# peterrum/dealii-multigrid

Measured on AMD Instinct MI355X. Metric: DoF/s per V-cycle, 3D octant p=4, higher is better.
Workload: dtype f64; 1 GPU; 3D octant (GeometryType quadrant) HMG-global p=4 FP64, NRefGlobal=8, SmootherDegree=3, coarse solver direct, f=1, zero Dirichlet (BASELINE.json configs[2]); n_dofs=137199985, n_cells=2127189, n_levels=9, parallelism=1 GPU, chebyshev_start_vector=deal.II's (i mod 11) - mean on the local numbering, fused_transfer_bricks=33509

## Files before the change

### dealii_multigrid_amd/csrc/kernels_apply.hpp

```cpp
#pragma once
#include "kernels_common.hpp"

namespace mgamd
{
#ifdef MGAMD_KERNEL_DEBUG
#define MGAMD_STAMP(k)                         \
  if (args.stamps && tid == 0)                 \
    args.stamps[(size_t)block * 8 + (k)] = wall_clock64();
#define MGAMD_ABLATED(bit) (args.ablate & (bit))
#else
#define MGAMD_STAMP(k)
#define MGAMD_ABLATED(bit) false
#endif

  template <typename T, int P, int B, int MODE, bool CONSTR = false, bool WAVE = false>
  __device__ __forceinline__ void
  lattice_apply_body(const ApplyArgs<T, P> &args, const uint32_t block, const uint32_t nblocks, unsigned char *smem_raw)
  {
    static_assert(!WAVE || (B == 1 && !CONSTR), "wave-scoped slots: single cells");
    using G  = Geo<P, B, WAVE ? 64 : 256>;
    using IM = InteriorMap<P, B, WAVE ? 64 : 256>;
    T *bufA = reinterpret_cast<T *>(smem_raw);
    T *bufB = bufA + G::SPW * G::N3;

// ... 196 lines not shown
      {
        any_hanging = __syncthreads_or((int)(fm_early != 0)) != 0;
        if (any_hanging)
          brick_constraint_passes<T, P, B, BLOCK>(bufA, args.m, tid, nslots, args.g.fmask + slot0, false, G::ROUNDS == 1 ? &fm_line : nullptr);
      }
    MGAMD_STAMP(5)

    if (!MGAMD_ABLATED(1))
      {
        if constexpr (G::ROUNDS == 1)
          lattice_sweeps<T, P, B, BLOCK, NoHook, false, false, WAVE>(bufA, bufB, args.m, tid, nslots, &h_mine, NoHook(), true);
        else
          lattice_sweeps<T, P, B, BLOCK, NoHook, false, false, WAVE>(bufA, bufB, args.m, tid, nslots, args.g.h + slot0);
      }
    MGAMD_STAMP(6)

    if (B == 1 && any_hanging)
      hanging_passes<T, P, WAVE>(bufA, args.m, sl, u, v, act, mask, true);
    if constexpr (brick_may_be_constrained(B, CONSTR))
      if (any_hanging)
        brick_constraint_passes<T, P, B, BLOCK>(bufA, args.m, tid, nslots, args.g.fmask + slot0, true, G::ROUNDS == 1 ? &fm_line : nullptr);
    MGAMD_STAMP(2)

    if (G::N_INT > 0 && !MGAMD_ABLATED(4))
      {
#pragma unroll
        for (int it = 0; it < ITER; ++it)
          if (const Ent e = ent(it); e.l >= 0)
            {
              const T ax = bufA[e.l];
              T       r;
              if (MODE == MODE_VMULT)
                r = ax;
              else if (MODE == MODE_RESIDUAL)
                r = bv[it] - ax;
              else
                {
                  const T dv  = CLOSED_DINV ? interior_dinv(it) : dvm[CLOSED_DINV ? 0 : it];
                  const T xov = MODE == MODE_CHEB_SECOND ? args.epi.c0 * dv * bv[it] : xo[it];
                  r           = xg[it] + args.epi.f1 * (xg[it] - xov) + args.epi.f2 * dv * (bv[it] - ax);
                }
              if (MODE == MODE_CHEB)
                store_result(args.epi, e.g, r);
              else
                NT_STORE(r, &args.epi.out[e.g]);
            }
      }
    MGAMD_STAMP(3)
    if (!MGAMD_ABLATED(2))
      {
#pragma unroll
        for (int it = 0; it < ITERS; ++it)
          if (spos[it] >= 0 && sgi[it] < args.scatter_limit)
            atomic_add(&args.tail_acc[sgi[it] - args.n_interior], bufA[spos[it]]);
      }
#ifdef MGAMD_KERNEL_DEBUG
    if (args.stamps)
      {
        __builtin_amdgcn_s_waitcnt(0);
        slot_sync<WAVE>();
        MGAMD_STAMP(4)
      }
#endif
  }

  template <typename T, int P, int B, int MODE_, bool CONSTR = false>
  __device__ __forceinline__ void
  lattice_apply_persistent_body(const ApplyArgs<T, P> &args, const uint32_t w, const uint32_t stride, unsigned char *smem_raw)
  {
    using G  = Geo<P, B>;
    using IM = InteriorMap<P, B>;
    static_assert(G::SPW == 1 && G::N_INT > 0, "persistent workgroups: one slot per workgroup");
    constexpr int  MODE   = base_mode(MODE_);
    constexpr bool FUSE_R = MODE_ == MODE_RESIDUAL_RESTRICT, FUSE_P = MODE_ == MODE_CHEB_PROLONGATE, FUSE = FUSE_R || FUSE_P;
    static_assert(!FUSE || (!CONSTR && B >= 2 && G::ABLOCK == 256), "fused transfers: plain bricks, 256 threads");
    constexpr int BC = B >= 2 ? B / 2 : 1, NC = P * BC + 1, NC3 = NC * NC * NC;
    T *bufA = reinterpret_cast<T *>(smem_raw);
    T *bufB = bufA + G::N3;
    T *dtab = bufB + G::N3;
    T *Etab = dtab + 2 * P * P * P + 1;
    constexpr bool FACE_PASSES = CONSTR && P >= 2 && B > 2 && face_table_words<P, B>() > 0 && G::N * (G::N - 2) <= G::ABLOCK;

    constexpr int BLOCK = G::ABLOCK;
    constexpr int ITER  = (G::N_INT + BLOCK - 1) / BLOCK;
    constexpr int ITERS = (G::N_SHELL + BLOCK - 1) / BLOCK;
    constexpr int ITC   = FUSE ? (NC3 + BLOCK - 1) / BLOCK : 1;
    constexpr int P3    = P * P * P;
    static_assert(!FUSE || 2 * ITERS <= 15, "two flag bits per shell entry in a 16-bit word");

    const int      tid = threadIdx.x;
    const uint32_t n   = args.g.n_slots;
    if (w >= n)
      return;

    if constexpr (FACE_PASSES)
      for (int t = tid; t < (2 * P + 1) * (P + 1); t += BLOCK)
        {
          const int a = t / (P + 1), b = t % (P + 1);
          Etab[t]     = a <= P ? args.m.I0[a * (P + 1) + b] : args.m.I1[(a - P) * (P + 1) + b];
        }
    if (is_cheb(MODE))
      {
        for (int t = tid; t < P3; t += BLOCK)
          {
            const int tt[3] = {t % P, (t / P) % P, t / (P * P)};
            T         m[3], k[3];
#pragma unroll
// ... 304 lines not shown
                  }
                __syncthreads();
                for (int l = tid; l < NC * NC; l += BLOCK)
                  {
                    const int b0 = (l / NC) * G::N + l % NC;
#pragma unroll
                    for (int i = 0; i < G::N; ++i)
                      rin[i] = bufA[b0 + i * G::N * G::N];
                    line_embed_sym_T<T, P, BC>(args.fused.Eh, rin, rout);
#pragma unroll
                    for (int i = 0; i < NC; ++i)
                      bufB[l + i * NC * NC] = rout[i];
                  }
                __syncthreads();
#pragma unroll
                for (int it = 0; it < ITC; ++it)
                  if (tid + it * BLOCK < NC3 && cgi[it] != DEV_INVALID)
                    atomic_add(&args.fused.coarse[cgi[it]], bufB[tid + it * BLOCK]);
              }
          }
        else
          {
            InteriorWalk wk = walk0;
#pragma unroll
            for (int it = 0; it < ITER; ++it, wk.next())
              if (has_entry(it))
                {
                  const uint32_t g  = base + (uint32_t)(tid + it * BLOCK);
                  const T        ax = bufA[wk.pos()];
                  T              r;
                  if (MODE == MODE_VMULT)
                    r = ax;
                  else if (MODE == MODE_RESIDUAL)
                    r = bv[it] - ax;
                  else
                    {
                      const T dv  = interior_dinv(wk.type());
                      const T xov = MODE == MODE_CHEB_SECOND ? args.epi.c0 * dv * bv[it] : xo[it];
                      const T xv  = x_from_b ? args.epi.c0 * dv * bv[it] : xg[it];
                      if (FUSE_P)
                        r = xv + args.epi.f2 * dv * (bv[it] - ax);
                      else
                        r = xv + args.epi.f1 * (xv - xov) + args.epi.f2 * dv * (bv[it] - ax);
                    }
                  if (MODE == MODE_CHEB && !FUSE_P)
                    store_result(args.epi, g, r);
                  else
                    NT_STORE(r, &args.epi.out[g]);
                }
            MGAMD_STAMP(3)
#pragma unroll
            for (int it = 0; it < ITERS; ++it)
              if (spos[it] >= 0 && sgi[it] < args.scatter_limit)
                atomic_add(&args.tail_acc[sgi[it] - args.n_interior], bufA[spos[it]]);
          }
        MGAMD_STAMP(4)
        if (!has_next)
          break;
        v    = vn;
        slot  = slotn;
        base  = basen;
        hcur  = hn;
        fmcur = fmn;
        flcur = fln;
#pragma unroll
        for (int it = 0; it < ITC; ++it)
          {
            cgi[it]  = cgn[it];
            cval[it] = cvaln[it];
          }
#pragma unroll
        for (int it = 0; it < ITERS; ++it)
          {
            sgi[it]  = sgn[it];
            sval[it] = svaln[it];
            sb[it]   = sbn[it];
          }
#pragma unroll
        for (int it = 0; it < ITER; ++it)
          xg[it] = xgn[it];
        __syncthreads();
      }
  }
#undef MGAMD_STAMP
#undef MGAMD_ABLATED

  template <typename T, int P, int B, int MODE, bool CONSTR = false>
  __global__ void
  __launch_bounds__((Geo<P, B>::ABLOCK), (Geo<P, B>::ROUNDS > 1 ? 2 : (B == 1 ? 6 : (B == 2 ? 4 : 1)))) lattice_apply_kernel(const ApplyArgs<T, P> args)
  {
    extern __shared__ __align__(16) unsigned char smem_raw[];
    lattice_apply_body<T, P, B, MODE, CONSTR>(args, blockIdx.x, gridDim.x, smem_raw);
  }

  constexpr int CELL_WAVES = 4;
  template <typename T, int P>
  constexpr size_t
  cell_wave_lds()
  {
    using G = Geo<P, 1, 64>;
    return (((2 * (size_t)G::SPW * G::N3 + 2 * P * P * P + G::SPW) * sizeof(T) + 15) / 16) * 16;
  }
  template <typename T, int P, int MODE>
  __device__ __forceinline__ void
  cell_waves_body(const ApplyArgs<T, P> &args, const uint32_t block, const uint32_t nblocks, unsigned char *smem_raw)
  {
    const uint32_t wave = threadIdx.x >> 6;
// ... 70 lines not shown
        a.stamps          = nullptr;
        lattice_apply_persistent_body<T, P, B, base_mode(MODE), true>(a, blockIdx.x - args.n_wg_plain, gridDim.x - args.n_wg_plain, smem_raw);
      }
  }

  template <typename T, int P>
  struct SmallSlotsArgs
  {
    ApplyArgs<T, P> a;
    SlotGroupDev    g_cells;
    uint32_t        n_wg_bricks;
  };
  template <typename T, int P, int MODE>
  __global__ void
  __launch_bounds__(256, 4) lattice_apply_small_kernel(const SmallSlotsArgs<T, P> args)
  {
    extern __shared__ __align__(16) unsigned char smem_raw[];
    if (blockIdx.x < args.n_wg_bricks)
      lattice_apply_body<T, P, 2, MODE>(args.a, blockIdx.x, args.n_wg_bricks, smem_raw);
    else
      {
        ApplyArgs<T, P> a = args.a;
        a.g               = args.g_cells;
        a.stamps          = nullptr;
        cell_waves_body<T, P, MODE>(a, blockIdx.x - args.n_wg_bricks, gridDim.x - args.n_wg_bricks, smem_raw);
      }
  }

  struct CellClusterDev
  {
    const uint32_t *uniq_ptr;
    const uint32_t *uniq_idx;
    const uint16_t *loc;
    const uint16_t *mask;
    const double   *h;
    uint32_t        n_slots;
    uint32_t        max_uniq;
  };
  constexpr int CLUSTER_CELLS = 256;
  constexpr int CLUSTER_ITERS = 8;

  template <typename T>
  struct ClusterArgs
  {
    CellClusterDev c;
    Mats<1, T>     m;
    const T       *src;
    T             *tail_acc;
    uint32_t       n_interior;
    const T *b, *dinv;
    T        c0;
    int      from_b;
    uint32_t cluster_offset;
  };

  template <typename T, bool TRANSPOSE>
  __device__ __forceinline__ void
  hanging_in_registers_p1(T (&x)[8], const uint32_t mask, const Mats<1, T> &m)
  {
    const int  cx = mask & 1, cy = (mask >> 1) & 1, cz = (mask >> 2) & 1;
    const bool fx = (mask >> 3) & 1, fy = (mask >> 4) & 1, fz = (mask >> 5) & 1;
    const bool ex = (mask >> 6) & 1, ey = (mask >> 7) & 1, ez = (mask >> 8) & 1;
#pragma unroll
    for (int dd = 0; dd < 3; ++dd)
      {
        const int d = TRANSPOSE ? 2 - dd : dd;
#pragma unroll
        for (int v = 0; v < 2; ++v)
#pragma unroll
          for (int u = 0; u < 2; ++u)
            {
              bool on;
              int  c;
              if (d == 0)
                {
                  const bool ou = u == cy, ov = v == cz;
                  on            = (fy && ou) || (fz && ov) || (ex && ou && ov);
                  c             = cx;
                }
              else if (d == 1)
                {
                  const bool ou = u == cx, ov = v == cz;
                  on            = (fx && ou) || (fz && ov) || (ey && ou && ov);
                  c             = cy;
                }
              else
                {
                  const bool ou = u == cx, ov = v == cy;
                  on            = (fx && ou) || (fy && ov) || (ez && ou && ov);
                  c             = cz;
                }
              const int i0 = d == 0 ? (v * 2 + u) * 2 : (d == 1 ? v * 4 + u : v * 2 + u);
              const int i1 = i0 + (d == 0 ? 1 : (d == 1 ? 2 : 4));
              if (on)
                {
                  const T *w       = c ? m.I1 : m.I0;
                  const T       a0 = x[i0], a1 = x[i1];
                  if (TRANSPOSE)
                    {
                      x[i0] = T(w[0]) * a0 + T(w[2]) * a1;
                      x[i1] = T(w[1]) * a0 + T(w[3]) * a1;
                    }
                  else
                    {
                      x[i0] = T(w[0]) * a0 + T(w[1]) * a1;
                      x[i1] = T(w[2]) * a0 + T(w[3]) * a1;
// ... 65 lines not shown
    T             x[8];
#pragma unroll
    for (int i = 0; i < 8; ++i)
      {
        l[i] = (lw4[i / 2] >> (16 * (i % 2))) & 0xFFFFu;
        x[i] = (act && l[i] != 0xFFFFu) ? U[l[i]] : T(0);
      }
    if (mask >> 3)
      hanging_in_registers_p1<T, false>(x, mask, a.m);
    const T M0 = T(a.m.M[0]), M1 = T(a.m.M[1]), M2 = T(a.m.M[2]), M3 = T(a.m.M[3]);
    const T K0 = T(a.m.K[0]), K1 = T(a.m.K[1]), K2 = T(a.m.K[2]), K3 = T(a.m.K[3]);
    T       A[8], Bv[8];
#pragma unroll
    for (int q = 0; q < 4; ++q)
      {
        const T r0 = x[q], r1 = x[q + 4];
        A[q]       = M0 * r0 + M1 * r1;
        A[q + 4]   = M2 * r0 + M3 * r1;
        Bv[q]      = K0 * r0 + K1 * r1;
        Bv[q + 4]  = K2 * r0 + K3 * r1;
      }
#pragma unroll
    for (int q = 0; q < 4; ++q)
      {
        const int i0 = (q & 1) + 4 * (q >> 1);
        const T   a0 = A[i0], a1 = A[i0 + 2], b0 = Bv[i0], b1 = Bv[i0 + 2];
        A[i0]        = M0 * a0 + M1 * a1;
        A[i0 + 2]    = M2 * a0 + M3 * a1;
        Bv[i0]       = K0 * a0 + K1 * a1 + M0 * b0 + M1 * b1;
        Bv[i0 + 2]   = K2 * a0 + K3 * a1 + M2 * b0 + M3 * b1;
      }
#pragma unroll
    for (int q = 0; q < 4; ++q)
      {
        const T a0 = A[2 * q], a1 = A[2 * q + 1], b0 = Bv[2 * q], b1 = Bv[2 * q + 1];
        x[2 * q]     = h * (K0 * a0 + K1 * a1 + M0 * b0 + M1 * b1);
        x[2 * q + 1] = h * (K2 * a0 + K3 * a1 + M2 * b0 + M3 * b1);
      }
    if (mask >> 3)
      hanging_in_registers_p1<T, true>(x, mask, a.m);
    if (act)
      {
#pragma unroll
        for (int i = 0; i < 8; ++i)
          if (l[i] != 0xFFFFu)
            atomic_add(&Acc[l[i]], x[i]);
      }
    __syncthreads();
#pragma unroll
    for (int k = 0; k < CLUSTER_ITERS; ++k)
      {
        const int j = tid + k * CLUSTER_CELLS;
        if (j < nu)
          atomic_add(&a.tail_acc[gi[k] - a.n_interior], Acc[j]);
      }
  }

  template <typename T>
  __global__ void
  __launch_bounds__(CLUSTER_CELLS) cell_cluster_apply_kernel(const ClusterArgs<T> a)
  {
    extern __shared__ __align__(16) unsigned char smem_raw[];
    cell_cluster_body<T>(a, blockIdx.x, gridDim.x, smem_raw);
  }

  template <typename T>
  struct P1SmallArgs
  {
    ApplyArgs<T, 1> a;
    ClusterArgs<T>  c;
    uint32_t        n_wg_bricks;
  };
  template <typename T, int MODE>
  __global__ void
  __launch_bounds__(256) lattice_cluster_kernel(const P1SmallArgs<T> args)
  {
    extern __shared__ __align__(16) unsigned char smem_raw[];
    if (blockIdx.x < args.n_wg_bricks)
      lattice_apply_body<T, 1, 8, MODE>(args.a, blockIdx.x, args.n_wg_bricks, smem_raw);
    else
      cell_cluster_body<T>(args.c, blockIdx.x - args.n_wg_bricks, gridDim.x - args.n_wg_bricks, smem_raw);
  }

  template <typename T, int P, int B, bool CONSTR = false>
  __global__ void
  __launch_bounds__((Geo<P, B>::BLOCK)) lattice_diag_kernel(const ApplyArgs<T, P> args)
  {
    using G = Geo<P, B>;
    extern __shared__ __align__(16) unsigned char smem_raw[];
    T *bufA = reinterpret_cast<T *>(smem_raw);
    T *bufB = bufA + G::SPW * G::N3;
    T *bufD = bufB + G::SPW * G::N3;

    const int tid    = threadIdx.x;
    const int slot0  = blockIdx.x * G::SPW;
    const int nslots = min((int)G::SPW, (int)args.g.n_slots - slot0);
    const int sl     = tid / G::LINES;
    const int ln     = tid % G::LINES;
    const int u = ln % G::N, v = ln / G::N;
    const bool act = tid < G::SPW * G::LINES && sl < nslots;

    uint32_t mask = 0;
    T        h    = T(0);
    if (act)
      {
        h = T(args.g.h[slot0 + sl]);
        if (B == 1)
// ... 39 lines not shown
        if (any_hanging)
          for (int j = 0; j < G::N3; ++j)
            {
              for (int idx = tid; idx < G::SPW * G::N3; idx += G::BLOCK)
                bufA[idx] = (idx % G::N3) == j ? T(1) : T(0);
              __syncthreads();
              hanging_passes<T, P>(bufA, args.m, sl, u, v, act, mask, false);
              lattice_sweeps<T, P, B, G::BLOCK>(bufA, bufB, args.m, tid, nslots, args.g.h + slot0);
              hanging_passes<T, P>(bufA, args.m, sl, u, v, act, mask, true);
              if (act && ln == 0 && (mask >> 3))
                bufD[sl * G::N3 + j] = bufA[sl * G::N3 + j];
              __syncthreads();
            }
      }
    if constexpr (brick_may_be_constrained(B, CONSTR))
      {
        uint32_t fm = 0;
        if (args.g.fmask != nullptr && tid < nslots)
          fm = args.g.fmask[slot0 + tid];
        const bool any_family = __syncthreads_or((int)(fm != 0)) != 0;
        if (any_family)
          for (int s = 0; s < G::N_SHELL; ++s)
            {
              const int j = args.g.shell_pos[s];
              for (int idx = tid; idx < G::SPW * G::N3; idx += G::BLOCK)
                bufA[idx] = (idx % G::N3) == j ? T(1) : T(0);
              __syncthreads();
              brick_constraint_passes<T, P, B, G::BLOCK>(bufA, args.m, tid, nslots, args.g.fmask + slot0, false);
              lattice_sweeps<T, P, B, G::BLOCK>(bufA, bufB, args.m, tid, nslots, args.g.h + slot0);
              brick_constraint_passes<T, P, B, G::BLOCK>(bufA, args.m, tid, nslots, args.g.fmask + slot0, true);
              if (act && ln == 0 && args.g.fmask[slot0 + sl])
                bufD[sl * G::N3 + j] = bufA[sl * G::N3 + j];
              __syncthreads();
            }
      }
    if (G::N_INT > 0)
      for (int idx = tid; idx < nslots * G::N_INT; idx += G::BLOCK)
        {
          const int sl2 = idx / (G::N_INT > 0 ? G::N_INT : 1), i = idx % (G::N_INT > 0 ? G::N_INT : 1);
          const int x = i % (G::NI > 0 ? G::NI : 1), y = (i / (G::NI > 0 ? G::NI : 1)) % (G::NI > 0 ? G::NI : 1),
                    z = i / (G::NI > 0 ? G::NI * G::NI : 1);
          const T d = bufD[sl2 * G::N3 + ((z + 1) * G::N + (y + 1)) * G::N + x + 1];
          apply_epilogue<T, MODE_INVDIAG>(args.epi, args.g.interior_base[slot0 + sl2] + i, d);
        }
    for (int idx = tid; idx < nslots * G::N_SHELL; idx += G::BLOCK)
      {
        const int      sl2 = idx / G::N_SHELL, s = idx % G::N_SHELL;
        const uint32_t gi  = args.g.shell_idx[(size_t)(slot0 + sl2) * G::N_SHELL + s];
        if (gi < args.scatter_limit)
          atomic_add(&args.tail_acc[gi - args.n_interior], bufD[sl2 * G::N3 + args.g.shell_pos[s]]);
      }
  }

  template <typename T, int MODE_>
  __global__ void
  __launch_bounds__(256) tail_kernel(T *__restrict__ tail_acc, uint32_t n_interior, uint32_t n_tail, uint32_t n_rest, Epilogue<T> epi)
  {
    constexpr int  MODE   = base_mode(MODE_);
    constexpr bool FUSE_P = MODE_ == MODE_CHEB_PROLONGATE;
    constexpr int  U      = 4;
    const uint32_t total  = n_tail + n_rest;
    const uint32_t stride = gridDim.x * blockDim.x;
    __shared__ T   dtable[256];
    const bool     coded = is_cheb(MODE) && epi.dinv_code != nullptr;
    if (coded)
      {
        dtable[threadIdx.x] = epi.dinv_table[threadIdx.x];
        __syncthreads();
      }
    for (uint32_t i0 = blockIdx.x * blockDim.x + threadIdx.x; i0 < total; i0 += U * stride)
      {
        T ax[U], xv[U], xo[U], bv[U], dv[U];
#pragma unroll
        for (int u = 0; u < U; ++u)
          {
            const uint32_t i  = i0 + u * stride;
            const uint32_t gi = n_interior + i;
            ax[u] = xv[u] = xo[u] = bv[u] = dv[u] = T(0);
            if (i < total)
              {
                if (MODE != MODE_INVDIAG && MODE != MODE_CHEB_FIRST && (is_cheb(MODE) || i >= n_tail))
                  {
                    if (FUSE_P && i < n_tail && NT_LOAD(&epi.xs_flag[i]))
                      {
                        xv[u] = NT_LOAD(&epi.xs[gi]);
                        epi.x_inout[gi] = xv[u];
                      }
                    else
                      xv[u] = NT_LOAD(&epi.x[gi]);
                  }
                ax[u] = i < n_tail ? tail_acc[i] : xv[u];
                if (MODE == MODE_RESIDUAL || is_cheb(MODE))
                  bv[u] = NT_LOAD(&epi.b[gi]);
                if (is_cheb(MODE))
                  {
                    if (MODE == MODE_CHEB && epi.xold)
                      xo[u] = NT_LOAD(&epi.xold[gi]);
                    if (coded)
                      {
                        const uint32_t c = NT_LOAD(&epi.dinv_code[i]);
                        dv[u]            = c != 255u ? dtable[c] : epi.dinv[gi];
                      }
                    else
                      dv[u] = epi.dinv[gi];
                  }
              }
          }
#pragma unroll
        for (int u = 0; u < U; ++u)
          {
            const uint32_t i  = i0 + u * stride;
            const uint32_t gi = n_interior + i;
            if (i < total)
              {
                if (i < n_tail)
                  NT_STORE(T(0), &tail_acc[i]);
                if (MODE == MODE_CHEB_FIRST || MODE == MODE_CHEB_SECOND)
                  {
                    const T x1 = epi.c0 * dv[u] * bv[u];
                    if (MODE == MODE_CHEB_FIRST)
                      {
                        xv[u] = x1;
                        if (i >= n_tail)
                          ax[u] = x1;
                      }
                    else
                      xo[u] = x1;
                  }
                if (MODE == MODE_VMULT)
                  NT_STORE(ax[u], &epi.out[gi]);
                else if (MODE == MODE_RESIDUAL)
                  NT_STORE(bv[u] - ax[u], &epi.out[gi]);
                else if (is_cheb(MODE))
                  {
                    const T r = xv[u] + epi.f1 * (xv[u] - xo[u]) + epi.f2 * dv[u] * (bv[u] - ax[u]);
                    if (MODE_ == MODE_CHEB)
                      store_result(epi, gi, r);
                    else
                      NT_STORE(r, &epi.out[gi]);
                  }
                else
                  epi.out[gi] = (i < n_tail && fabs((double)ax[u]) > 1.0e-10) ? T(1) / ax[u] : T(1);
              }
          }
      }
  }

}
```

### dealii_multigrid_amd/csrc/kernels_common.hpp

```cpp
#pragma once
#include <hip/hip_runtime.h>
#include <stdint.h>

namespace mgamd
{
  constexpr uint32_t DEV_INVALID = 0xFFFFFFFFu;

#ifndef MGAMD_NO_NT_STREAMS
#define NT_LOAD(p) __builtin_nontemporal_load(p)
#define NT_STORE(v, p) __builtin_nontemporal_store(v, p)
#else
#define NT_LOAD(p) (*(p))
#define NT_STORE(v, p) (*(p) = (v))
#endif

  __device__ __forceinline__ uint32_t
  xcd_contiguous(uint32_t b, uint32_t n)
  {
    const uint32_t k = b & 7u, q = n >> 3, r = n & 7u;
    return k * q + (k < r ? k : r) + (b >> 3);
  }

  template <int P, typename S = double>
  struct Mats
// ... 66 lines not shown
    T        f1, f2;
    T        c0;
    const uint8_t *dinv_code  = nullptr;
    const T       *dinv_table = nullptr;
    const uint8_t *xs_flag = nullptr;
    const T       *xs      = nullptr;
    T             *x_inout = nullptr;
    double *out_wide = nullptr;
  };
  template <typename T>
  __device__ __forceinline__ void
  store_result(const Epilogue<T> &e, const uint32_t g, const T r)
  {
    if (sizeof(T) == 4 && e.out_wide != nullptr)
      __builtin_nontemporal_store((double)r, &e.out_wide[g]);
    else
      __builtin_nontemporal_store(r, &e.out[g]);
  }
  constexpr bool
  is_cheb(int mode)
  {
    return mode == MODE_CHEB || mode == MODE_CHEB_FIRST || mode == MODE_CHEB_SECOND;
  }

  template <typename T, int MODE>
  __device__ __forceinline__ void
  apply_epilogue(const Epilogue<T> &e, uint32_t gi, T Ax)
  {
    if (MODE == MODE_VMULT)
      e.out[gi] = Ax;
    else if (MODE == MODE_RESIDUAL)
      e.out[gi] = e.b[gi] - Ax;
    else if (MODE == MODE_CHEB)
      {
        const T xv = e.x[gi];
        const T xo = e.xold ? e.xold[gi] : T(0);
        e.out[gi]  = xv + e.f1 * (xv - xo) + e.f2 * e.dinv[gi] * (e.b[gi] - Ax);
      }
    else
      e.out[gi] = (fabs((double)Ax) > 1.0e-10) ? T(1) / Ax : T(1);
  }

  __device__ __forceinline__ void
  atomic_add(double *p, double v)
  {
    unsafeAtomicAdd(p, v);
  }
  __device__ __forceinline__ void
  atomic_add(float *p, float v)
  {
    unsafeAtomicAdd(p, v);
  }

  template <typename T, int P, int B>
  __device__ __forceinline__ void
  line_mult(const T *__restrict__ Mc, const T (&in)[P * B + 1], T (&out)[P * B + 1])
  {
#pragma unroll
    for (int i = 0; i < P * B + 1; ++i)
      out[i] = T(0);
#pragma unroll
    for (int c = 0; c < B; ++c)
#pragma unroll
      for (int a = 0; a <= P; ++a)
#pragma unroll
        for (int b = 0; b <= P; ++b)
          out[c * P + a] += T(Mc[a * (P + 1) + b]) * in[c * P + b];
  }

  template <typename T, int P>
  struct EvenOdd
  {
    static constexpr int NH = (P + 2) / 2, NO = (P + 1) / 2;
    T                    e[NH], o[NO];
    __device__ __forceinline__ void
    split(const T *x)
    {
#pragma unroll
      for (int j = 0; j < NO; ++j)
        {
          e[j] = x[j] + x[P - j];
          o[j] = x[j] - x[P - j];
        }
      if (NH > NO)
        e[NH - 1] = x[NH - 1];
    }
    template <bool ACC>
    __device__ __forceinline__ void
    apply(const T *__restrict__ Ae, const T *__restrict__ Ao, const EvenOdd &x)
    {
#pragma unroll
      for (int i = 0; i < NH; ++i)
        {
          T acc = ACC ? e[i] : T(0);
#pragma unroll
          for (int j = 0; j < NH; ++j)
            acc += T(Ae[i * NH + j]) * x.e[j];
          e[i] = acc;
        }
#pragma unroll
      for (int i = 0; i < NO; ++i)
        {
          T acc = ACC ? o[i] : T(0);
#pragma unroll
          for (int j = 0; j < NO; ++j)
            acc += T(Ao[i * NO + j]) * x.o[j];
// ... 826 lines not shown
```

### dealii_multigrid_amd/csrc/level_operator.hpp

```cpp
#pragma once
#include "runtime.hpp"
#include "kernels.hpp"

#include <cmath>
#include <cstring>
#include <map>
#include <mutex>
#include <type_traits>
#include <unordered_map>

namespace mgamd
{
  inline int
  grid_for(size_t n)
  {
    size_t g = (n + 255) / 256;
    if (g > 2048)
      g = 2048;
    if (g < 1)
      g = 1;
    return (int)g;
  }

  template <typename T>
// ... 365 lines not shown
                           halo->sh_owner_src.p, nsh);
      HIP_CHECK(hipGetLastError());
    }
    void
    exchange_add_tail(mgamd_vec &v) override
    {
      if (v.n != n_dofs())
        throw std::invalid_argument("exchange_add_tail: vector size mismatch");
      exchange_add_raw(v.as<T>() + tables->n_interior);
    }
    double
    dot_raw_global(const T *x, const T *y)
    {
      if (!comm)
        return dot_raw(ctx, x, y, (size_t)n_dofs());
      const double local = dot_raw(ctx, x, y, (size_t)tables->n_interior + tables->n_tail_owned);
      return comm->allreduce_sum_host(local, ctx->stream);
    }
    double
    dot(const mgamd_vec &x, const mgamd_vec &y) override
    {
      if (x.n != n_dofs() || y.n != n_dofs())
        throw std::invalid_argument("dot: vector size mismatch");
      return dot_raw_global(x.as<T>(), y.as<T>());
    }

    template <int P>
    Mats<P, T>
    mats() const
    {
      Mats<P, T> m;
      const int n = P + 1;
      for (int i = 0; i < n * n; ++i)
        {
          m.M[i]  = tables->fe.M[i];
          m.K[i]  = tables->fe.K[i];
          m.I0[i] = tables->fe.I[0][i];
          m.I1[i] = tables->fe.I[1][i];
        }
      constexpr int NH = Mats<P>::NH, NO = Mats<P>::NO;
      auto          eo = [&](const double *A, T *Ae, T *Ao) {
        for (int i = 0; i < NH; ++i)
          for (int j = 0; j < NH; ++j)
            Ae[i * NH + j] = (j < NO) ? 0.5 * (A[i * n + j] + A[i * n + P - j]) : A[i * n + j];
        for (int i = 0; i < NO; ++i)
          for (int j = 0; j < NO; ++j)
            Ao[i * NO + j] = 0.5 * (A[i * n + j] - A[i * n + P - j]);
      };
      eo(tables->fe.M.data(), m.Me, m.Mo);
      eo(tables->fe.K.data(), m.Ke, m.Ko);
      return m;
    }

    ClusterArgs<T>
    cluster_args(const GroupDev<T> &g, const T *src, const Epilogue<T> &epi, bool first)
    {
      ClusterArgs<T> a;
      a.c          = g.cluster_view();
      a.m          = mats<1>();
      a.src        = src;
      a.tail_acc   = tail_acc.p;
      a.n_interior = tables->n_interior;
      a.b          = epi.b;
      a.dinv       = epi.dinv;
      a.c0         = epi.c0;
      a.from_b     = first ? 1 : 0;
      a.cluster_offset = 0;
      return a;
    }

    void
    launch_clusters(hipStream_t st, const GroupDev<T> &g, const T *src, const Epilogue<T> &epi, bool first, uint32_t cluster_begin = 0,
                    uint32_t cluster_end = 0xFFFFFFFFu)
    {
      ClusterArgs<T> a;
      a.c          = g.cluster_view();
      a.m          = mats<1>();
      a.src        = src;
      a.tail_acc   = tail_acc.p;
      a.n_interior = tables->n_interior;
      a.b          = epi.b;
      a.dinv       = epi.dinv;
      a.c0         = epi.c0;
      a.from_b     = first ? 1 : 0;
      a.cluster_offset = 0;
      const uint32_t n_cl = (uint32_t)((g.n_slots + CLUSTER_CELLS - 1) / CLUSTER_CELLS);
      cluster_end         = std::min(cluster_end, n_cl);
      if (cluster_begin >= cluster_end)
        return;
      a.cluster_offset    = cluster_begin;
      const uint32_t grid = cluster_end - cluster_begin;
      hipLaunchKernelGGL(cell_cluster_apply_kernel<T>, grid, CLUSTER_CELLS, 2 * (size_t)std::max<uint32_t>(g.max_uniq, 1) * sizeof(T), st, a);
      HIP_CHECK(hipGetLastError());
    }

    template <int P, int B, int MODE>
    void
    launch_pair(hipStream_t st, const ApplyArgs<T, P> &a, GroupDev<T> *g_constrained)
    {
      using G = Geo<P, B>;
      BrickPairArgs<T, P> pa;
      pa.a             = a;
      pa.g_constrained = g_constrained->view();
      pa.n_wg_plain    = (uint32_t)((a.g.n_slots + G::SPW - 1) / G::SPW);
      const uint32_t n_wg_c = (uint32_t)((g_constrained->n_slots + G::SPW - 1) / G::SPW);
      const size_t   lds    = (2 * (size_t)G::SPW * G::N3 + 2 * P * P * P + G::SPW + face_table_words<P, B>()) * sizeof(T);
      if constexpr (G::SPW == 1 && G::N_INT > 0 && G::ROUNDS > 1)
        if (use_persistent<T, P>())
          {
            const int resident = resident_workgroups(ctx);
            uint32_t  np = pa.n_wg_plain, nc = n_wg_c;
            if ((int)(np + nc) > resident)
              {
                np = 0;
                nc = (uint32_t)resident;
              }
            pa.n_wg_plain = np;
            auto kern     = lattice_apply_persistent_pair_kernel<T, P, B, MODE>;
            ensure_dynamic_lds(ctx, reinterpret_cast<const void *>(kern), lds);
            hipLaunchKernelGGL(kern, np + nc, G::ABLOCK, lds, st, pa);
            HIP_CHECK(hipGetLastError());
            return;
          }
      if constexpr (MODE != base_mode(MODE))
        throw std::runtime_error("fused transfers need the persistent brick kernel");
      else
        {
          auto kern = lattice_apply_pair_kernel<T, P, B, MODE>;
          ensure_dynamic_lds(ctx, reinterpret_cast<const void *>(kern), lds);
          hipLaunchKernelGGL(kern, pa.n_wg_plain + n_wg_c, G::ABLOCK, lds, st, pa);
          HIP_CHECK(hipGetLastError());
        }
    }

    template <int P, int MODE>
    void
    launch_fused(hipStream_t st, ApplyArgs<T, P> &a, size_t begin, GroupDev<T> *partner_constrained, const FusedTransferHost<T> &f)
    {
// ... 13 lines not shown
              if (std::fabs(f.E[(2 * P - ar) * (P + 1) + (P - b)] - f.E[ar * (P + 1) + b]) > 1e-14)
                throw std::runtime_error("fused transfer: the 1D embedding is not centro-symmetric");
          a.fused.coarse  = f.coarse;
          a.fused.x_inout = f.x_inout;
          a.fused.scratch = f.scratch;
          if (partner_constrained)
            {
              if constexpr (P == 1)
                return launch_pair<P, B, MODE>(st, a, partner_constrained);
              throw std::runtime_error("brick pair launch: size not instantiated");
            }
          const size_t lds      = (2 * (size_t)G::N3 + 2 * P * P * P + 1 + face_table_words<P, B>()) * sizeof(T);
          const int    resident = resident_workgroups(ctx, persistent_wgs_per_cu<T, P>());
          auto         kern     = lattice_apply_persistent_kernel<T, P, B, MODE>;
          ensure_dynamic_lds(ctx, reinterpret_cast<const void *>(kern), lds);
          hipLaunchKernelGGL(kern, std::min((int)a.g.n_slots, resident), G::ABLOCK, lds, st, a);
          HIP_CHECK(hipGetLastError());
        }
      else
        throw std::runtime_error("fused transfers: degree without 17-point lattice kernel");
    }

    template <int P, int MODE_>
    void
    launch_group(hipStream_t st, ApplyArgs<T, P> &a, GroupDev<T> *g, GroupDev<T> *partner_cells, GroupDev<T> *partner_clusters,
                 const T *src, const Epilogue<T> &epi, bool diag, size_t begin, size_t end, GroupDev<T> *partner_constrained = nullptr,
                 const FusedTransferHost<T> *fused = nullptr)
    {
      constexpr int MODE = base_mode(MODE_);
      a.g      = (begin == 0 && end == g->n_slots) ? g->view() : g->view(begin, end);
      if constexpr (MODE_ != MODE)
        if (fused && fused->group >= 0 && g == groups[fused->group].get())
          return launch_fused<P, MODE_>(st, a, begin, partner_constrained, *fused);
      if (partner_constrained)
        {
          if constexpr (P == 1)
            {
              if (g->B == 16)
                return launch_pair<P, 16, MODE>(st, a, partner_constrained);
              if (g->B == 8)
                return launch_pair<P, 8, MODE>(st, a, partner_constrained);
            }
          throw std::runtime_error("brick pair launch: size not instantiated");
        }
      a.stamps = (stamps.p && g->B == prof_B && !g->constrained && MODE == stamp_mode && !diag && begin == 0) ? stamps.p : nullptr;
      if (partner_clusters)
        {
          if constexpr (P == 1)
            {
              using G8 = Geo<1, 8>;
              GroupDev<T>   *gc = partner_clusters;
              P1SmallArgs<T> sa;
              sa.a           = a;
              sa.c           = cluster_args(*gc, src, epi, MODE == MODE_CHEB_FIRST);
              sa.n_wg_bricks = (uint32_t)((g->n_slots + G8::SPW - 1) / G8::SPW);
              const uint32_t n_wg_cl = (uint32_t)((gc->n_slots + CLUSTER_CELLS - 1) / CLUSTER_CELLS);
              const size_t   lds     = std::max((2 * (size_t)G8::SPW * G8::N3 + 2 + G8::SPW) * sizeof(T),
                                          2 * (size_t)std::max<uint32_t>(gc->max_uniq, 1) * sizeof(T));
              hipLaunchKernelGGL((lattice_cluster_kernel<T, MODE>), sa.n_wg_bricks + n_wg_cl, 256, lds, st, sa);
              HIP_CHECK(hipGetLastError());
            }
        }
      else if (P == 1 && !diag && g->has_clusters())
        launch_clusters(st, *g, src, epi, MODE == MODE_CHEB_FIRST);
      else if (partner_cells)
        {
          if constexpr (P >= 2)
            {
              using G2 = Geo<P, 2>;
              using G1 = Geo<P, 1>;
              GroupDev<T>         *g1 = partner_cells;
              SmallSlotsArgs<T, P> sa;
              sa.a           = a;
              sa.g_cells     = g1->view();
              sa.n_wg_bricks = (uint32_t)((g->n_slots + G2::SPW - 1) / G2::SPW);
              using GW = Geo<P, 1, 64>;
              const uint32_t n_w        = (uint32_t)((g1->n_slots + GW::SPW - 1) / GW::SPW);
              const uint32_t n_wg_cells = (n_w + CELL_WAVES - 1) / CELL_WAVES;
              const size_t   lds        = std::max((2 * (size_t)G2::SPW * G2::N3 + 2 * P * P * P + G2::SPW) * sizeof(T), CELL_WAVES * cell_wave_lds<T, P>());
              (void)sizeof(G1);
              hipLaunchKernelGGL((lattice_apply_small_kernel<T, P, MODE>), sa.n_wg_bricks + n_wg_cells, 256, lds, st, sa);
              HIP_CHECK(hipGetLastError());
            }
        }
      else
        dispatch_B<T, P, MODE>(ctx, st, g->B, g->constrained, a, diag);
    }

    template <int MODE>
    void
    launch_tail(hipStream_t st, uint32_t begin, uint32_t end, bool with_rest, const Epilogue<T> &epi_in, bool diag)
    {
      const uint32_t n_rest = with_rest ? tables->n_dofs - tables->n_interior - end : 0;
      const uint32_t n_t    = end - begin + n_rest;
      if (!n_t)
        return;
      Epilogue<T> epi = epi_in;
      if (epi.dinv_code)
        epi.dinv_code += begin;
      if (diag)
        hipLaunchKernelGGL((tail_kernel<T, MODE_INVDIAG>), grid_for(n_t), 256, 0, st, tail_acc.p + begin, tables->n_interior + begin, end - begin,
                           n_rest, epi);
      else
        hipLaunchKernelGGL((tail_kernel<T, MODE>), grid_for(n_t), 256, 0, st, tail_acc.p + begin, tables->n_interior + begin, end - begin, n_rest,
                           epi);
      HIP_CHECK(hipGetLastError());
    }

    enum EdgeMode
    {
      EDGE_OUT  = 0,
      EDGE_ROWS = 1,
      EDGE_IN   = 2
    };

    template <int P, int MODE>
    void
    apply_P(const T *src, const Epilogue<T> &epi, bool diag, double words, int edge_mode, const FusedTransferHost<T> *fused);

    template <int MODE>
    void
    apply(const T *src, const Epilogue<T> &epi, bool diag = false, double words = 0, int edge_mode = EDGE_OUT,
          const FusedTransferHost<T> *fused = nullptr)
    {
      constexpr bool FUSED_MODE = MODE != base_mode(MODE);
      if (FUSED_MODE && (!fused || fused->group < 0 || !fused_transfer_supported<T>(p)))
        throw std::runtime_error("fused transfer pass without fused tables");
      switch (p)
        {
          case 1:
            apply_P<1, MODE>(src, epi, diag, words, edge_mode, fused);
            break;
          case 2:
            apply_P<2, MODE>(src, epi, diag, words, edge_mode, fused);
            break;
          case 3:
            if constexpr (!FUSED_MODE)
              apply_P<3, MODE>(src, epi, diag, words, edge_mode, fused);
            break;
          case 4:
            apply_P<4, MODE>(src, epi, diag, words, edge_mode, fused);
            break;
          default:
            throw std::runtime_error("degree not instantiated");
        }
    }

    void
    vmult_raw(T *dst, const T *src)
    {
      Epilogue<T> e{dst, src, nullptr, nullptr, nullptr, T(0), T(0), T(0)};
      apply<MODE_VMULT>(src, e);
    }
    void
    residual_raw(T *t, const T *b, const T *x)
    {
      Epilogue<T> e{t, x, nullptr, b, nullptr, T(0), T(0), T(0)};
      apply<MODE_RESIDUAL>(x, e, false, 0, tables->n_edge ? EDGE_IN : EDGE_OUT);
    }
// ... 145 lines not shown
```

### dealii_multigrid_amd/csrc/level_operator_apply.hpp

```cpp
#pragma once
#include "level_operator.hpp"

namespace mgamd
{
  template <typename T>
  template <int P, int MODE>
  void
  LevelOperator<T>::apply_P(const T *src, const Epilogue<T> &epi, bool diag, double words, int edge_mode, const FusedTransferHost<T> *fused)
  {
    constexpr int BASE = base_mode(MODE);
    ApplyArgs<T, P> a;
    const uint32_t  first_edge = tables->n_interior + tables->n_tail;
    a.gather_limit  = first_edge + (edge_mode == EDGE_IN ? tables->n_edge : 0);
    a.scatter_limit = first_edge + (edge_mode != EDGE_OUT ? tables->n_edge : 0);
    const uint32_t tail_end = tables->n_tail + (edge_mode != EDGE_OUT ? tables->n_edge : 0);
    a.m          = mats<P>();
    a.src        = src;
    a.tail_acc   = tail_acc.p;
    a.n_interior = tables->n_interior;
    a.ablate     = ablate;
    a.stamps     = nullptr;
    a.epi        = epi;
    GroupDev<T> *g2 = nullptr, *g1 = nullptr;
    if (P >= 2 && !diag && merge_small)
      for (auto &g : groups)
        {
          if (g->n_slots && g->B == 2)
            g2 = g.get();
          else if (g->n_slots && g->B == 1)
            g1 = g.get();
        }
    const bool merged = g2 && g1;
    GroupDev<T> *g8 = nullptr, *gc = nullptr;
    if (P == 1 && !diag && merge_small)
      for (auto &g : groups)
        {
          if (g->n_slots && g->B == 8 && g->B != prof_B && !g->constrained)
            g8 = g.get();
          else if (g->n_slots && g->B == 1 && g->has_clusters())
            gc = g.get();
        }
    const bool merged_p1 = g8 && gc;

    if (halo && !diag && halo_overlap)
      {
        auto halo_end = [&](const GroupDev<T> &g) -> size_t {
          size_t nh = g.n_halo;
          if (P == 1 && g.has_clusters())
            nh = std::min(g.n_slots, (nh + CLUSTER_CELLS - 1) / CLUSTER_CELLS * CLUSTER_CELLS);
          return nh;
        };
        auto launch_range = [&](GroupDev<T> *g, size_t begin, size_t end) {
          if (begin >= end)
            return;
          if (P == 1 && g->has_clusters())
            launch_clusters(ctx->stream, *g, src, epi, BASE == MODE_CHEB_FIRST, (uint32_t)(begin / CLUSTER_CELLS),
                            (uint32_t)((end + CLUSTER_CELLS - 1) / CLUSTER_CELLS));
          else
            {
              a.g = g->view(begin, end);
              if (MODE != BASE && fused && fused->group >= 0 && g == groups[fused->group].get())
                {
                  if constexpr (MODE != BASE)
                    launch_fused<P, MODE>(ctx->stream, a, begin, nullptr, *fused);
                }
              else
                dispatch_B<T, P, BASE>(ctx, ctx->stream, g->B, g->constrained, a, diag);
            }
        };
        size_t n_interior_slots = 0;
        for (auto &g : groups)
          n_interior_slots += g->n_slots - halo_end(*g);
        if (n_interior_slots > 0)
          {
            for (auto &g : groups)
              launch_range(g.get(), 0, halo_end(*g));
            ctx->order_after(ctx->side, ctx->stream);
            exchange_add_raw(tail_acc.p, ctx->side);
            for (auto &g : groups)
              launch_range(g.get(), halo_end(*g), g->n_slots);
            ctx->order_after(ctx->stream, ctx->side);
            launch_tail<MODE>(ctx->stream, 0, tail_end, true, epi, diag);
            return;
          }
      }
    const hipStream_t main = ctx->stream;
    auto prof_begin = [&](const GroupDev<T> &g) {
      const bool prof = ctx->profile && !diag && MODE == MODE_CHEB && !g.constrained && g.B == (ctx->prof_brick ? ctx->prof_brick : prof_B);
      if (prof)
        {
          if (ctx->prof_used == ctx->prof_events.size())
            {
              hipEvent_t e0, e1;
              HIP_CHECK(hipEventCreate(&e0));
              HIP_CHECK(hipEventCreate(&e1));
              ctx->prof_events.push_back({e0, e1});
            }
          HIP_CHECK(hipEventRecord(ctx->prof_events[ctx->prof_used].first, main));
        }
      return prof;
    };
    auto prof_end = [&](const GroupDev<T> &g, size_t n_slots) {
      HIP_CHECK(hipEventRecord(ctx->prof_events[ctx->prof_used].second, main));
      ++ctx->prof_used;
      const bool   closed_dinv = P == 1 || (g.N * g.N > 256 && use_persistent<T, P>());
      const double w_interior  = words - (closed_dinv ? 1.0 : 0.0);
      const double n1 = (double)(g.N - 1), n2 = (double)(g.N - 2);
      ctx->prof_bytes += sizeof(T) * (double)n_slots * (words * n2 * n2 * n2 + 2.0 * (n1 * n1 * n1 - n2 * n2 * n2));
      ctx->prof_bytes_moved += sizeof(T) * (double)n_slots * (w_interior * n2 * n2 * n2 + 2.0 * (n1 * n1 * n1 - n2 * n2 * n2));
    };
    auto constrained_partner = [&](GroupDev<T> *g) -> GroupDev<T> * {
      if (P != 1 || diag || !merge_small || g->constrained || g->B <= 2 || (merged_p1 && g == g8))
        return nullptr;
      for (auto &q : groups)
        if (q->constrained && q->B == g->B && q->n_slots)
          return q.get();
      return nullptr;
    };
    for (size_t gi = 0; gi < groups.size(); ++gi)
      {
        GroupDev<T> *g = groups[gi].get();
        if (!g->n_slots)
          continue;
        if ((merged && g == g1) || (merged_p1 && g == gc))
          continue;
        if (g->constrained && !diag && merge_small && P == 1)
          {
            bool has_plain = false;
            for (auto &q : groups)
              has_plain |= !q->constrained && q->B == g->B && q->n_slots && !(merged_p1 && q.get() == g8);
            if (has_plain)
              continue;
          }
        const bool prof = prof_begin(*g);
        launch_group<P, MODE>(main, a, g, (merged && g == g2) ? g1 : nullptr, (merged_p1 && g == g8) ? gc : nullptr, src, epi, diag, 0,
                              g->n_slots, constrained_partner(g), fused);
        if (prof)
          prof_end(*g, g->n_slots);
      }
    if (halo)
      exchange_add_raw(tail_acc.p);
    launch_tail<MODE>(main, 0, tail_end, true, epi, diag);
  }

}
```

Measured before the change: 14.83 billion DoF/s.

## Initialize tail outputs before cell kernels and scatter directly into output for vmult/residual

For vmult and residual modes without halo exchange, a tail-init kernel now writes the non-accumulated part of the output (b or zero) before the cell kernels run. The cell kernels then atomically add (or subtract) their shell contributions straight into the output vector instead of into a separate tail accumulator. This removes the reading and zeroing of the tail accumulator in the final tail pass and moves that pass ahead of the cell work. The cost is atomics on the large output vector rather than a compact accumulator, plus an aliasing check that falls back to the old path.

```diff
diff --git a/dealii_multigrid_amd/csrc/kernels_apply.hpp b/dealii_multigrid_amd/csrc/kernels_apply.hpp
--- a/dealii_multigrid_amd/csrc/kernels_apply.hpp
+++ b/dealii_multigrid_amd/csrc/kernels_apply.hpp
@@ -272,7 +272,7 @@
 #pragma unroll
         for (int it = 0; it < ITERS; ++it)
           if (spos[it] >= 0 && sgi[it] < args.scatter_limit)
-            atomic_add(&args.tail_acc[sgi[it] - args.n_interior], bufA[spos[it]]);
+            tail_scatter<T, MODE>(args.tail_acc, args.epi, args.n_interior, sgi[it], bufA[spos[it]]);
       }
 #ifdef MGAMD_KERNEL_DEBUG
     if (args.stamps)
@@ -683,7 +683,7 @@
 #pragma unroll
             for (int it = 0; it < ITERS; ++it)
               if (spos[it] >= 0 && sgi[it] < args.scatter_limit)
-                atomic_add(&args.tail_acc[sgi[it] - args.n_interior], bufA[spos[it]]);
+                tail_scatter<T, MODE>(args.tail_acc, args.epi, args.n_interior, sgi[it], bufA[spos[it]]);
           }
         MGAMD_STAMP(4)
         if (!has_next)
@@ -860,6 +860,8 @@
     T        c0;
     int      from_b;
     uint32_t cluster_offset;
+    T *out  = nullptr;
+    T  beta = T(1);
   };
 
   template <typename T, bool TRANSPOSE>
@@ -1031,7 +1033,12 @@
       {
         const int j = tid + k * CLUSTER_CELLS;
         if (j < nu)
-          atomic_add(&a.tail_acc[gi[k] - a.n_interior], Acc[j]);
+          {
+            if (a.tail_acc != nullptr)
+              atomic_add(&a.tail_acc[gi[k] - a.n_interior], Acc[j]);
+            else
+              atomic_add(&a.out[gi[k]], a.beta * Acc[j]);
+          }
       }
   }
 
@@ -1177,12 +1184,13 @@
       }
   }
 
-  template <typename T, int MODE_>
-  __global__ void
-  __launch_bounds__(256) tail_kernel(T *__restrict__ tail_acc, uint32_t n_interior, uint32_t n_tail, uint32_t n_rest, Epilogue<T> epi)
+  template <typename T, int MODE_, bool INIT>
+  __device__ __forceinline__ void
+  tail_body(T *__restrict__ tail_acc, uint32_t n_interior, uint32_t n_tail, uint32_t n_rest, const Epilogue<T> &epi)
   {
     constexpr int  MODE   = base_mode(MODE_);
     constexpr bool FUSE_P = MODE_ == MODE_CHEB_PROLONGATE;
+    static_assert(!INIT || tail_init_mode(MODE_), "tail_init_kernel: epilogues with beta = +-1 only");
     constexpr int  U      = 4;
     const uint32_t total  = n_tail + n_rest;
     const uint32_t stride = gridDim.x * blockDim.x;
@@ -1214,7 +1222,10 @@
                     else
                       xv[u] = NT_LOAD(&epi.x[gi]);
                   }
-                ax[u] = i < n_tail ? tail_acc[i] : xv[u];
+                if (i >= n_tail)
+                  ax[u] = xv[u];
+                else if (!INIT)
+                  ax[u] = tail_acc[i];
                 if (MODE == MODE_RESIDUAL || is_cheb(MODE))
                   bv[u] = NT_LOAD(&epi.b[gi]);
                 if (is_cheb(MODE))
@@ -1238,7 +1249,7 @@
             const uint32_t gi = n_interior + i;
             if (i < total)
               {
-                if (i < n_tail)
+                if (!INIT && i < n_tail)
                   NT_STORE(T(0), &tail_acc[i]);
                 if (MODE == MODE_CHEB_FIRST || MODE == MODE_CHEB_SECOND)
                   {
@@ -1252,23 +1263,40 @@
                     else
                       xo[u] = x1;
                   }
+                T r;
                 if (MODE == MODE_VMULT)
-                  NT_STORE(ax[u], &epi.out[gi]);
+                  r = ax[u];
                 else if (MODE == MODE_RESIDUAL)
-                  NT_STORE(bv[u] - ax[u], &epi.out[gi]);
+                  r = bv[u] - ax[u];
                 else if (is_cheb(MODE))
-                  {
-                    const T r = xv[u] + epi.f1 * (xv[u] - xo[u]) + epi.f2 * dv[u] * (bv[u] - ax[u]);
-                    if (MODE_ == MODE_CHEB)
-                      store_result(epi, gi, r);
-                    else
-                      NT_STORE(r, &epi.out[gi]);
-                  }
+                  r = xv[u] + epi.f1 * (xv[u] - xo[u]) + epi.f2 * dv[u] * (bv[u] - ax[u]);
                 else
-                  epi.out[gi] = (i < n_tail && fabs((double)ax[u]) > 1.0e-10) ? T(1) / ax[u] : T(1);
+                  r = (i < n_tail && fabs((double)ax[u]) > 1.0e-10) ? T(1) / ax[u] : T(1);
+                if (INIT && i < n_tail)
+                  epi.out[gi] = r;
+                else if (MODE_ == MODE_CHEB)
+                  store_result(epi, gi, r);
+                else if (MODE != MODE_INVDIAG)
+                  NT_STORE(r, &epi.out[gi]);
+                else
+                  epi.out[gi] = r;
               }
           }
       }
   }
 
+  template <typename T, int MODE_>
+  __global__ void
+  __launch_bounds__(256) tail_kernel(T *__restrict__ tail_acc, uint32_t n_interior, uint32_t n_tail, uint32_t n_rest, Epilogue<T> epi)
+  {
+    tail_body<T, MODE_, false>(tail_acc, n_interior, n_tail, n_rest, epi);
+  }
+
+  template <typename T, int MODE_>
+  __global__ void
+  __launch_bounds__(256) tail_init_kernel(uint32_t n_interior, uint32_t n_tail, uint32_t n_rest, Epilogue<T> epi)
+  {
+    tail_body<T, MODE_, true>(nullptr, n_interior, n_tail, n_rest, epi);
+  }
+
 }
diff --git a/dealii_multigrid_amd/csrc/kernels_common.hpp b/dealii_multigrid_amd/csrc/kernels_common.hpp
--- a/dealii_multigrid_amd/csrc/kernels_common.hpp
+++ b/dealii_multigrid_amd/csrc/kernels_common.hpp
@@ -142,6 +142,22 @@
     unsafeAtomicAdd(p, v);
   }
 
+  constexpr bool
+  tail_init_mode(int mode)
+  {
+    return mode == MODE_VMULT || mode == MODE_RESIDUAL || mode == MODE_RESIDUAL_RESTRICT;
+  }
+
+  template <typename T, int MODE>
+  __device__ __forceinline__ void
+  tail_scatter(T *tail_acc, const Epilogue<T> &e, const uint32_t n_interior, const uint32_t gi, const T v)
+  {
+    if (!tail_init_mode(MODE) || tail_acc != nullptr)
+      atomic_add(&tail_acc[gi - n_interior], v);
+    else
+      atomic_add(&e.out[gi], MODE == MODE_VMULT ? v : -v);
+  }
+
   template <typename T, int P, int B>
   __device__ __forceinline__ void
   line_mult(const T *__restrict__ Mc, const T (&in)[P * B + 1], T (&out)[P * B + 1])
diff --git a/dealii_multigrid_amd/csrc/level_operator.hpp b/dealii_multigrid_amd/csrc/level_operator.hpp
--- a/dealii_multigrid_amd/csrc/level_operator.hpp
+++ b/dealii_multigrid_amd/csrc/level_operator.hpp
@@ -441,9 +441,11 @@
       return m;
     }
 
+    template <int MODE>
     ClusterArgs<T>
-    cluster_args(const GroupDev<T> &g, const T *src, const Epilogue<T> &epi, bool first)
-    {
+    cluster_args(const GroupDev<T> &g, const T *src, const Epilogue<T> &epi, bool init)
+    {
+      const bool first = MODE == MODE_CHEB_FIRST;
       ClusterArgs<T> a;
       a.c          = g.cluster_view();
       a.m          = mats<1>();
@@ -455,13 +457,16 @@
       a.c0         = epi.c0;
       a.from_b     = first ? 1 : 0;
       a.cluster_offset = 0;
+      set_cluster_tail<MODE>(a, epi, init);
       return a;
     }
 
-    void
-    launch_clusters(hipStream_t st, const GroupDev<T> &g, const T *src, const Epilogue<T> &epi, bool first, uint32_t cluster_begin = 0,
+    template <int MODE>
+    void
+    launch_clusters(hipStream_t st, const GroupDev<T> &g, const T *src, const Epilogue<T> &epi, bool init, uint32_t cluster_begin = 0,
                     uint32_t cluster_end = 0xFFFFFFFFu)
     {
+      const bool first = MODE == MODE_CHEB_FIRST;
       ClusterArgs<T> a;
       a.c          = g.cluster_view();
       a.m          = mats<1>();
@@ -473,6 +478,7 @@
       a.c0         = epi.c0;
       a.from_b     = first ? 1 : 0;
       a.cluster_offset = 0;
+      set_cluster_tail<MODE>(a, epi, init);
       const uint32_t n_cl = (uint32_t)((g.n_slots + CLUSTER_CELLS - 1) / CLUSTER_CELLS);
       cluster_end         = std::min(cluster_end, n_cl);
       if (cluster_begin >= cluster_end)
@@ -592,7 +598,7 @@
               GroupDev<T>   *gc = partner_clusters;
               P1SmallArgs<T> sa;
               sa.a           = a;
-              sa.c           = cluster_args(*gc, src, epi, MODE == MODE_CHEB_FIRST);
+              sa.c           = cluster_args<MODE>(*gc, src, epi, a.tail_acc == nullptr);
               sa.n_wg_bricks = (uint32_t)((g->n_slots + G8::SPW - 1) / G8::SPW);
               const uint32_t n_wg_cl = (uint32_t)((gc->n_slots + CLUSTER_CELLS - 1) / CLUSTER_CELLS);
               const size_t   lds     = std::max((2 * (size_t)G8::SPW * G8::N3 + 2 + G8::SPW) * sizeof(T),
@@ -602,7 +608,7 @@
             }
         }
       else if (P == 1 && !diag && g->has_clusters())
-        launch_clusters(st, *g, src, epi, MODE == MODE_CHEB_FIRST);
+        launch_clusters<MODE>(st, *g, src, epi, a.tail_acc == nullptr);
       else if (partner_cells)
         {
           if constexpr (P >= 2)
@@ -645,6 +651,40 @@
         hipLaunchKernelGGL((tail_kernel<T, MODE>), grid_for(n_t), 256, 0, st, tail_acc.p + begin, tables->n_interior + begin, end - begin, n_rest,
                            epi);
       HIP_CHECK(hipGetLastError());
+    }
+
+    template <int MODE>
+    void
+    launch_tail_init(hipStream_t st, const Epilogue<T> &epi)
+    {
+      const uint32_t n_t = tables->n_dofs - tables->n_interior;
+      if (!n_t)
+        return;
+      hipLaunchKernelGGL((tail_init_kernel<T, MODE>), grid_for(n_t), 256, 0, st, tables->n_interior, tables->n_tail,
+                         n_t - tables->n_tail, epi);
+      HIP_CHECK(hipGetLastError());
+    }
+
+    template <int MODE>
+    bool
+    use_tail_init(const T *src, const Epilogue<T> &epi, bool diag, int edge_mode) const
+    {
+      static const bool off = getenv("MGAMD_NO_TAIL_INIT") != nullptr;
+      if (!tail_init_mode(MODE) || off || halo || diag || edge_mode != EDGE_OUT || !epi.out)
+        return false;
+      const size_t n     = n_dofs();
+      auto         apart = [&](const T *v) { return !v || v + n <= epi.out || epi.out + n <= v; };
+      return apart(src) && apart(epi.x) && apart(epi.b);
+    }
+    template <int MODE>
+    void
+    set_cluster_tail(ClusterArgs<T> &a, const Epilogue<T> &epi, bool init) const
+    {
+      if (!init)
+        return;
+      a.tail_acc = nullptr;
+      a.out      = epi.out;
+      a.beta     = MODE == MODE_VMULT ? T(1) : T(-1);
     }
 
     enum EdgeMode
diff --git a/dealii_multigrid_amd/csrc/level_operator_apply.hpp b/dealii_multigrid_amd/csrc/level_operator_apply.hpp
--- a/dealii_multigrid_amd/csrc/level_operator_apply.hpp
+++ b/dealii_multigrid_amd/csrc/level_operator_apply.hpp
@@ -16,7 +16,8 @@
     const uint32_t tail_end = tables->n_tail + (edge_mode != EDGE_OUT ? tables->n_edge : 0);
     a.m          = mats<P>();
     a.src        = src;
-    a.tail_acc   = tail_acc.p;
+    const bool init = use_tail_init<MODE>(src, epi, diag, edge_mode);
+    a.tail_acc   = init ? nullptr : tail_acc.p;
     a.n_interior = tables->n_interior;
     a.ablate     = ablate;
     a.stamps     = nullptr;
@@ -54,7 +55,7 @@
           if (begin >= end)
             return;
           if (P == 1 && g->has_clusters())
-            launch_clusters(ctx->stream, *g, src, epi, BASE == MODE_CHEB_FIRST, (uint32_t)(begin / CLUSTER_CELLS),
+            launch_clusters<BASE>(ctx->stream, *g, src, epi, false, (uint32_t)(begin / CLUSTER_CELLS),
                             (uint32_t)((end + CLUSTER_CELLS - 1) / CLUSTER_CELLS));
           else
             {
@@ -85,6 +86,9 @@
           }
       }
     const hipStream_t main = ctx->stream;
+    if constexpr (tail_init_mode(MODE))
+      if (init)
+        launch_tail_init<MODE>(main, epi);
     auto prof_begin = [&](const GroupDev<T> &g) {
       const bool prof = ctx->profile && !diag && MODE == MODE_CHEB && !g.constrained && g.B == (ctx->prof_brick ? ctx->prof_brick : prof_B);
       if (prof)
@@ -138,6 +142,8 @@
         if (prof)
           prof_end(*g, g->n_slots);
       }
+    if (init)
+      return;
     if (halo)
       exchange_add_raw(tail_acc.p);
     launch_tail<MODE>(main, 0, tail_end, true, epi, diag);
```

Result: no change. 14.91 billion DoF/s, median of 6 (+0.5%).
